# barlettacarmen/CrCNN

Hardware: NVIDIA B200
Metric: encrypted MNIST images/sec (higher is better)
Workload: dtype u64

## Files before the change

crcnn_b200/csrc/engine.cu:

```cuda
#include <cuda_runtime.h>
#include <dlfcn.h>
#include <algorithm>
#include <cstdlib>
#include <cstring>
#include <map>
#include <unordered_map>
#include <string>
#include <vector>

#include "../../include/crcnn_b200.h"
#include "kernels.cuh"
#include "params.h"
#include "tc_mac.cuh"
#include "tcn_mac.cuh"
#include "relin32.cuh"
#include "reenc.cuh"

using namespace crcnn;

namespace {

enum KernelClass {
    KC_NTT_FWD = 0, KC_NTT_INV, KC_MAC, KC_PLAIN_EXPAND, KC_POOL, KC_BN, KC_PLAIN_OP,
    KC_BEHZ_LIFT, KC_SQ_TENSOR, KC_BEHZ_FLOOR, KC_RELIN, KC_PROBE, KC_TC_SPLIT, KC_TC_MAC, KC_TCN_SPLIT, KC_TCN_MAC, KC_RELIN32, KC_REENC, KC_COUNT
// ... 1498 lines not shown
            e = launch_ntt_inv_tensor(ctx->dP, ctx->logn, ext, have_ntt ? src : nullptr, cur, KS, prod, fold, !lean, ctx->stream);
        }
        if (e == cudaSuccess) { ProfScope ps(ctx, KC_BEHZ_FLOOR, lp_bytes(ctx, (double)cur * 3 * (KS + ctx->K)),
                                                     (double)cur * 3 * n * (ctx->S * (ctx->K + 1) + ctx->S + ctx->K * ctx->S)); e = launch_behz_floor(ctx->hp.d, ctx->n, prod, cur, o->d + c0 * 3 * pw, ctx->stream, !lean); }
        if (e != cudaSuccess) rc = fail(ctx, CRCNN_ERR_CUDA, cudaGetErrorString(e));
    }
    dev_free(ctx, coef);
    dev_free(ctx, ext); dev_free(ctx, prod);
    if (rc) { crcnn_tensor_free(ctx, o); return rc; }
    *out3 = o;
    return CRCNN_OK;
}

int crcnn_relinearize(crcnn_ctx *ctx, crcnn_tensor *in3, crcnn_evk *evk, crcnn_tensor **out2) {
    if (!ctx) return CRCNN_ERR_INVALID_ARGUMENT;
    REQUIRE(in3 && evk && out2, "null argument");
    REQUIRE(in3->size == 3, "relinearize expects size-3 ciphertexts");
    int total_digits = 0;
    for (int i = 0; i < ctx->K; i++) {
        int bits = 0; for (uint64_t v = ctx->hp.d.tab[i].mod.q; v; v >>= 1) bits++;
        REQUIRE(evk->digits[i] * evk->dbc >= bits, "not enough evaluation keys");
        total_digits += evk->digits[i];
    }
    REQUIRE(total_digits <= 63, "too many key digits for 128-bit lazy accumulation");
    CU(cudaSetDevice(ctx->device));
    int rc = ensure_domain(ctx, in3, 0);
    if (rc) return rc;
    crcnn_tensor *o = nullptr;
    rc = new_tensor(ctx, in3->count, 2, 0, &o);
    if (rc) return rc;
    const size_t pw = poly_words(ctx);
    if (evk->has_r32 && ctx->relin_mode == 1) {
        const Relin32Consts &c = evk->r32.c;
        const size_t per_ct = relin32_scratch_bytes(ctx->n, ctx->K, c);
        const long step = std::max<long>(1, std::min<long>(std::min<long>(in3->count, 200000), (long)((2ull << 30) / per_ct)));
        void *scratch = nullptr;
        rc = dev_alloc(ctx, (size_t)step * per_ct, &scratch);
        if (rc) { crcnn_tensor_free(ctx, o); return rc; }
        for (long c0 = 0; c0 < in3->count && !rc; c0 += step) {
            const long cnt = std::min<long>(step, in3->count - c0);
            ProfScope ps(ctx, KC_RELIN32, lp_bytes(ctx, (double)cnt * 5 * ctx->K),
                         lp_bfly(ctx, (double)cnt * (c.D + 2 * ctx->K) * c.S3));
            cudaError_t e = relin32_run(ctx->dP, ctx->logn, ctx->K, evk->r32, in3->d + c0 * 3 * pw, o->d + c0 * 2 * pw, cnt, scratch, ctx->stream);
            if (e != cudaSuccess) rc = fail(ctx, CRCNN_ERR_CUDA, cudaGetErrorString(e));
        }
        dev_free(ctx, scratch);
        if (rc) { crcnn_tensor_free(ctx, o); return rc; }
        *out2 = o;
        return CRCNN_OK;
    }
    RelinArgs a{};
    a.evk = evk->d; a.dbc = evk->dbc;
    for (int i = 0; i < MAXK; i++) { a.key_off[i] = evk->key_off[i]; a.digits[i] = evk->digits[i]; }
    const size_t per_ct = (size_t)(1 + total_digits + 2) * pw * 8;
    const long step = std::max<long>(1, std::min<long>(in3->count, (long)((2ull << 30) / per_ct)));
    uint64_t *scratch = nullptr;
    rc = dev_alloc(ctx, (size_t)step * per_ct, (void **)&scratch);
    if (rc) { crcnn_tensor_free(ctx, o); return rc; }
    a.dsc = scratch;
    a.dig = scratch + (size_t)step * pw;
    a.acc = a.dig + (size_t)step * total_digits * pw;
    for (long c0 = 0; c0 < in3->count && !rc; c0 += step) {
        a.count = std::min<long>(step, in3->count - c0);
        a.in3 = in3->d + c0 * 3 * pw;
        a.out = o->d + c0 * 2 * pw;
        cudaError_t e;
        { ProfScope ps(ctx, KC_RELIN, lp_bytes(ctx, (double)a.count * 3 * ctx->K), lp_bfly(ctx, (double)a.count * total_digits * ctx->K)); e = launch_relin(ctx->dP, ctx->logn, ctx->K, a, ctx->stream); }
        if (e == cudaSuccess) {
            ProfScope ps(ctx, KC_NTT_INV, 2 * lp_bytes(ctx, (double)a.count * 2 * ctx->K) + lp_bytes(ctx, (double)a.count * 2 * ctx->K), lp_bfly(ctx, (double)a.count * 2 * ctx->K));
            e = launch_ntt_grouped(ctx->dP, ctx->logn, a.out, a.count * 2 * ctx->K, 0, ctx->K, true, ctx->K, 0, ctx->stream, a.acc, a.in3,
                                   2 * ctx->K, 3 * ctx->K);
        }
        if (e != cudaSuccess) rc = fail(ctx, CRCNN_ERR_CUDA, cudaGetErrorString(e));
    }
    dev_free(ctx, scratch);
    if (rc) { crcnn_tensor_free(ctx, o); return rc; }
// ... 476 lines not shown
```

crcnn_b200/csrc/relin32.cu:

```cuda
#include "relin32.cuh"
#include "kernels.cuh"
#include "devcfg.cuh"
#include "modarith.cuh"
#include <cmath>
#include <cstdlib>
#include <vector>

namespace crcnn {
namespace {

const uint32_t kAuxPrimes[R32_MAXP] = {1073643521u, 1073479681u, 1073184769u, 1073053697u};

uint32_t mulm(uint32_t a, uint32_t b, uint32_t p) { return (uint32_t)((uint64_t)a * b % p); }
uint32_t powm(uint32_t a, uint64_t e, uint32_t p) {
    uint32_t r = 1;
    for (; e; e >>= 1, a = mulm(a, a, p))
        if (e & 1) r = mulm(r, a, p);
    return r;
}
uint32_t invm(uint32_t a, uint32_t p) { return powm(a % p, p - 2, p); }
uint32_t shoup_companion(uint32_t w, uint32_t p) { return (uint32_t)(((uint64_t)w << 32) / p); }
uint32_t bitrev32(uint32_t v, int bits) {
    uint32_t r = 0;
    for (int i = 0; i < bits; i++) r |= ((v >> i) & 1u) << (bits - 1 - i);
// ... 108 lines not shown
    fwd_last_stage<NG, 3>(x, t4, p, twop, G);
    fwd_last_stage<NG, 4>(x, t4, p, twop, G);
}

template <int NG, int S>
__device__ __forceinline__ void inv_first_stage(uint32_t (&x)[32], const uint4 *__restrict__ t4, uint32_t p, uint32_t twop, int G) {
    constexpr int B = 5;
#pragma unroll
    for (int l2 = 0; l2 < (1 << (B - 2 - S)); l2++) {
        const uint4 W = __ldg(t4 + (16 - (16 >> S) + l2) * NG + G);
#pragma unroll
        for (int a = 0; a < (1 << S); a++) {
            const int i0 = ((2 * l2) << (S + 1)) + a, i1 = ((2 * l2 + 1) << (S + 1)) + a;
            gs32(x[i0], x[i0 + (1 << S)], W.x, W.y, p, twop);
            gs32(x[i1], x[i1 + (1 << S)], W.z, W.w, p, twop);
        }
    }
}

template <int NG>
__device__ __forceinline__ void inv_first32(uint32_t (&x)[32], const uint4 *__restrict__ t4, const uint2 *__restrict__ t1, uint32_t p,
                                            uint32_t twop, int G) {
    inv_first_stage<NG, 0>(x, t4, p, twop, G);
    inv_first_stage<NG, 1>(x, t4, p, twop, G);
    inv_first_stage<NG, 2>(x, t4, p, twop, G);
    inv_first_stage<NG, 3>(x, t4, p, twop, G);
    {
        const uint2 W = __ldg(t1 + G);
#pragma unroll
        for (int a = 0; a < 16; a++) gs32(x[a], x[a + 16], W.x, W.y, p, twop);
    }
}

template <int LOGN, int B, int GLOG, bool INV>
__device__ __forceinline__ void pass32(uint32_t *sm, const uint2 *__restrict__ tw, uint32_t p) {
    constexpr int N = 1 << LOGN, g = 1 << GLOG, TH = Plan32<LOGN>::THREADS;
    if constexpr (GLOG == 0) {
        static_assert(B == 5, "the contiguous pass takes 5 stages");
        constexpr int NG = N >> 5;
        const uint4 *t4 = reinterpret_cast<const uint4 *>(tw);
        const uint2 *t1 = tw + 30 * NG;
#pragma unroll 1
        for (int G = threadIdx.x; G < NG; G += TH) {
            uint4 *row = reinterpret_cast<uint4 *>(sm + G * 36);
            uint32_t x[32];
#pragma unroll
            for (int m = 0; m < 8; m++) {
                const uint4 v = row[m];
                x[4 * m] = v.x; x[4 * m + 1] = v.y; x[4 * m + 2] = v.z; x[4 * m + 3] = v.w;
            }
            if (INV) inv_first32<NG>(x, t4, t1, p, 2 * p, G);
            else fwd_last32<NG>(x, t4, t1, p, 2 * p, G);
#pragma unroll
            for (int m = 0; m < 8; m++) row[m] = make_uint4(x[4 * m], x[4 * m + 1], x[4 * m + 2], x[4 * m + 3]);
        }
    } else {
        static_assert(GLOG >= 5, "strided passes need gaps that are multiples of 32 words");
        constexpr int PSTR = g + (g >> 5) * 4;
#pragma unroll 1
        for (int G = threadIdx.x; G < (N >> B); G += TH) {
            const int blk = G >> GLOG, o = G & (g - 1);
            uint32_t *col = sm + pad32((blk << (GLOG + B)) + o);
            uint32_t x[1 << B];
#pragma unroll
            for (int k = 0; k < (1 << B); k++) x[k] = col[k * PSTR];
            if (INV) inv_group32<B>(x, tw, p, 2 * p, N >> (GLOG + 1), blk);
            else fwd_group32<B>(x, tw, p, 2 * p, (N >> (GLOG + B)) + blk);
#pragma unroll
            for (int k = 0; k < (1 << B); k++) col[k * PSTR] = x[k];
        }
    }
}

template <int LOGN>
__device__ __forceinline__ void ntt32_forward(uint32_t *sm, const uint2 *__restrict__ w, const uint2 *__restrict__ wl, uint32_t p) {
    using P = Plan32<LOGN>;
    constexpr int b0 = P::bits(0), b1 = P::NP > 1 ? P::bits(1) : 0;
    pass32<LOGN, b0, LOGN - b0, false>(sm, w, p);
    __syncthreads();
    if constexpr (P::NP > 1) {
        pass32<LOGN, b1, LOGN - b0 - b1, false>(sm, w, p);
        __syncthreads();
    }
    pass32<LOGN, 5, 0, false>(sm, wl, p);
    __syncthreads();
}

template <int LOGN>
__device__ __forceinline__ void ntt32_inverse(uint32_t *sm, const uint2 *__restrict__ iw, const uint2 *__restrict__ iwl, uint32_t p) {
    using P = Plan32<LOGN>;
    constexpr int b0 = P::bits(0), b1 = P::NP > 1 ? P::bits(1) : 0;
    pass32<LOGN, 5, 0, true>(sm, iwl, p);
    __syncthreads();
    if constexpr (P::NP > 1) {
        pass32<LOGN, b1, 5, true>(sm, iw, p);
        __syncthreads();
    }
    pass32<LOGN, b0, LOGN - b0, true>(sm, iw, p);
    __syncthreads();
}

template <int LOGN, int RANGE>
__device__ __forceinline__ void store32_canonical(const uint32_t *sm, uint32_t *__restrict__ dst, uint32_t p) {
    for (int i = threadIdx.x * 4; i < (1 << LOGN); i += Plan32<LOGN>::THREADS * 4) {
        uint4 v = *reinterpret_cast<const uint4 *>(sm + pad32(i));
        if (RANGE == 4) { v.x = csub(v.x, 2 * p); v.y = csub(v.y, 2 * p); v.z = csub(v.z, 2 * p); v.w = csub(v.w, 2 * p); }
        v.x = csub(v.x, p); v.y = csub(v.y, p); v.z = csub(v.z, p); v.w = csub(v.w, p);
        *reinterpret_cast<uint4 *>(dst + i) = v;
    }
}

__global__ void __launch_bounds__(256)
r32_scale_kernel(const DeviceParams *__restrict__ P, const Relin32Consts *__restrict__ cp, const uint64_t *__restrict__ in3,
                 uint16_t *__restrict__ planes) {
    const int n = P->n, K = P->K;
    const long pw = (long)K * n;
    const long ct = blockIdx.x;
    const long lw = ((long)blockIdx.y * 256 + threadIdx.x) * 2;
    const int i = (int)(lw / n), e = (int)(lw - (long)i * n);
    const ulonglong2 c2 = __ldg(reinterpret_cast<const ulonglong2 *>(in3 + (ct * 3 + 2) * pw + lw));
    const Mod mod = P->tab[i].mod;
    const uint64_t f = P->inv_qhat[i];
    const uint64_t v0 = mulmod(c2.x, f, mod), v1 = mulmod(c2.y, f, mod);
    const int dbc = cp->dbc, D = cp->D;
    const uint32_t mask = (1u << dbc) - 1;
    for (int d = cp->dfirst[i]; d < D && cp->dprime[d] == i; d++) {
        const int sh = cp->dshift[d];
        const uint32_t lo = (uint32_t)(v0 >> sh) & mask, hi = (uint32_t)(v1 >> sh) & mask;
        *reinterpret_cast<uint32_t *>(planes + (ct * D + d) * n + e) = lo | (hi << 16);
    }
}

template <int LOGN>
__global__ void __launch_bounds__(Plan32<LOGN>::THREADS, Plan32<LOGN>::MIN_CTAS)
r32_digits_kernel(const uint16_t *__restrict__ planes, const Relin32Consts *__restrict__ cp, uint32_t *__restrict__ dig) {
    extern __shared__ uint4 sm32v[];
    uint32_t *sm32 = reinterpret_cast<uint32_t *>(sm32v);
    constexpr int N = 1 << LOGN;
    const long b = blockIdx.x;
    const int S3 = cp->S3;
    const int s = (int)(b % S3);
    const long cd = b / S3;
    const uint32_t p = cp->p[s];
    const uint2 *w = cp->w[s];
    const uint16_t *src = planes + cd * N;
    for (int i = threadIdx.x * 8; i < N; i += Plan32<LOGN>::THREADS * 8) {
        const uint4 v = __ldg(reinterpret_cast<const uint4 *>(src + i));
        uint4 *dst = reinterpret_cast<uint4 *>(sm32 + pad32(i));
        dst[0] = make_uint4(v.x & 0xffffu, v.x >> 16, v.y & 0xffffu, v.y >> 16);
        dst[1] = make_uint4(v.z & 0xffffu, v.z >> 16, v.w & 0xffffu, v.w >> 16);
    }
    __syncthreads();
    ntt32_forward<LOGN>(sm32, w, cp->wl[s], p);
    store32_canonical<LOGN, 4>(sm32, dig + b * N, p);
}

struct KeyMap {
    long key_off[MAXK];
    uint32_t ninv[R32_MAXP];
};

template <int LOGN>
__global__ void __launch_bounds__(Plan32<LOGN>::THREADS, Plan32<LOGN>::MIN_CTAS)
r32_key_kernel(const uint64_t *__restrict__ coef, KeyMap km, const Relin32Consts *__restrict__ cp, int K, uint32_t *__restrict__ keys) {
    extern __shared__ uint4 sm32v[];
    uint32_t *sm32 = reinterpret_cast<uint32_t *>(sm32v);
    constexpr int N = 1 << LOGN;
    const long b = blockIdx.x;
    const int S3 = cp->S3, D = cp->D;
    const int s = (int)(b % S3);
    const int o = (int)((b / S3) % (2 * K));
    const int d = (int)(b / ((long)S3 * 2 * K));
    const int pi = o / K, j = o % K;
    const uint32_t p = cp->p[s];
    const uint64_t *src = coef + km.key_off[cp->dprime[d]] + ((long)(2 * (cp->dshift[d] / cp->dbc) + pi) * K + j) * N;
    for (int e = threadIdx.x; e < N; e += blockDim.x) sm32[pad32(e)] = (uint32_t)(__ldg(src + e) % p);
    __syncthreads();
    ntt32_forward<LOGN>(sm32, cp->w[s], cp->wl[s], p);
    uint32_t *dst = keys + (((long)s * D + d) * 2 * K + o) * N;
    const uint32_t ninv = km.ninv[s];
    for (int e = threadIdx.x; e < N; e += blockDim.x) {
        const uint32_t v = csub(csub(sm32[pad32(e)], 2 * p), p);
        dst[e] = (uint32_t)((uint64_t)v * ninv % p);
    }
}

__device__ __forceinline__ uint32_t red64_32(uint64_t x, uint64_t mu, uint32_t p) {
    const uint32_t r = (uint32_t)x - (uint32_t)__umul64hi(x, mu) * p;
    return csub(csub(r, 2 * p), p);
}
__device__ __forceinline__ void madwide(uint64_t &acc, uint32_t a, uint32_t b) {
    asm("mad.wide.u32 %0, %1, %2, %0;" : "+l"(acc) : "r"(a), "r"(b));
}

template <int T, int OC, int EW>
__global__ void __launch_bounds__(256)
r32_mac_kernel(const uint32_t *__restrict__ dig, const uint32_t *__restrict__ keys, const Relin32Consts *__restrict__ cp, int n,
               long count, int cpb, uint32_t *__restrict__ acc) {
    extern __shared__ uint4 sm32v[];
    uint32_t *ksm = reinterpret_cast<uint32_t *>(sm32v);
    constexpr int LANES = 256 / EW;
    const int el = threadIdx.x % EW, lane = threadIdx.x / EW;
    const int e = blockIdx.x * EW + el;
    const int s = blockIdx.y;
    const long ctb = (long)blockIdx.z * cpb;
    const long cte = min(ctb + cpb, count);
    const uint32_t p = cp->p[s];
    const uint64_t mu = cp->mu[s];
    const int D = cp->D, S3 = cp->S3;
    {
        const uint32_t *kg = keys + (long)s * D * OC * n + blockIdx.x * EW;
// ... 114 lines not shown
#pragma unroll
                for (int u = 0; u < CPS; u++) {
                    a[u][0] = red64_32(a[u][0], mu, p);
                    a[u][1] = red64_32(a[u][1], mu, p);
                }
            }
        }
#pragma unroll
        for (int u = 0; u < CPS; u++) {
            const long ct = ctb + (long)st * CPS + u;
            if (ct < cte) {
                uint32_t *ap = acc + ((ct * OC + og * 2) * S3 + s) * n + e0 + el;
                ap[0] = red64_32(a[u][0], mu, p);
                ap[(long)S3 * n] = red64_32(a[u][1], mu, p);
            }
        }
    }
}

template <int LOGN>
__global__ void __launch_bounds__(Plan32<LOGN>::THREADS, Plan32<LOGN>::MIN_CTAS)
r32_intt_kernel(const Relin32Consts *__restrict__ cp, uint32_t *__restrict__ acc) {
    extern __shared__ uint4 sm32v[];
    uint32_t *sm32 = reinterpret_cast<uint32_t *>(sm32v);
    constexpr int N = 1 << LOGN;
    const long b = blockIdx.x;
    const int s = (int)(b % cp->S3);
    const uint32_t p = cp->p[s];
    const uint2 *iw = cp->iw[s];
    uint32_t *poly = acc + b * N;
    for (int i = threadIdx.x * 4; i < N; i += Plan32<LOGN>::THREADS * 4)
        *reinterpret_cast<uint4 *>(sm32 + pad32(i)) = *reinterpret_cast<const uint4 *>(poly + i);
    __syncthreads();
    ntt32_inverse<LOGN>(sm32, iw, cp->iwl[s], p);
    store32_canonical<LOGN, 2>(sm32, poly, p);
}

struct CrtConsts {
    uint32_t p[R32_MAXP], half[R32_MAXP], ginv[R32_MAXP][R32_MAXP], ginvp[R32_MAXP][R32_MAXP];
    uint64_t c[R32_MAXP], csh[R32_MAXP], Pmodq, q;
};
template <int S3>
__device__ __forceinline__ uint64_t crt_one(const uint32_t (&r)[R32_MAXP], const CrtConsts &k) {
    uint32_t a[S3];
#pragma unroll
    for (int s = 0; s < S3; s++) {
        uint32_t t = r[s];
#pragma unroll
        for (int i = 0; i < s; i++) {
            const uint32_t ai = csub(a[i], k.p[s]);
            t = csub(shoup32(t + k.p[s] - ai, k.ginv[s][i], k.ginvp[s][i], k.p[s]), k.p[s]);
        }
        a[s] = t;
    }
    uint64_t v = a[0];
    bool neg = false, decided = false;
#pragma unroll
    for (int s = S3 - 1; s >= 0; s--) {
        if (s > 0) v += mulshoup_lazy((uint64_t)a[s], k.c[s], k.csh[s], k.q);
        if (!decided && a[s] != k.half[s]) { neg = a[s] > k.half[s]; decided = true; }
    }
    v = v >= 4 * k.q ? v - 4 * k.q : v;
    v = v >= 2 * k.q ? v - 2 * k.q : v;
    v = v >= k.q ? v - k.q : v;
    if (neg) v = submod(v, k.Pmodq, k.q);
    return v;
}

template <int S3>
__global__ void __launch_bounds__(256)
r32_crt_kernel(const DeviceParams *__restrict__ P, const Relin32Consts *__restrict__ cp, const uint32_t *__restrict__ acc,
               const uint64_t *__restrict__ in3, uint64_t *__restrict__ out) {
    const int n = P->n, K = P->K;
    const int e = (blockIdx.y * 256 + threadIdx.x) * 2;
    const int o = (int)(blockIdx.x % (unsigned)(2 * K));
    const long ct = blockIdx.x / (unsigned)(2 * K);
    const int pi = o / K, j = o % K;
    CrtConsts k;
#pragma unroll
    for (int s = 0; s < S3; s++) {
        k.p[s] = cp->p[s];
        k.half[s] = cp->half[s];
        k.c[s] = cp->cmodq[j][s];
        k.csh[s] = cp->cmodq_sh[j][s];
#pragma unroll
        for (int i = 0; i < s; i++) {
            k.ginv[s][i] = cp->ginv[s][i];
            k.ginvp[s][i] = cp->ginvp[s][i];
        }
    }
    k.Pmodq = cp->Pmodq[j];
    k.q = P->tab[j].mod.q;
    const uint32_t *r = acc + ((ct * 2 * K + o) * S3) * n + e;
    uint32_t r0[R32_MAXP], r1[R32_MAXP];
#pragma unroll
    for (int s = 0; s < S3; s++) {
        const uint2 v = __ldg(reinterpret_cast<const uint2 *>(r + (long)s * n));
        r0[s] = v.x;
        r1[s] = v.y;
    }
    const long w = (long)j * n + e;
    const ulonglong2 c = __ldg(reinterpret_cast<const ulonglong2 *>(in3 + (ct * 3 + pi) * (long)K * n + w));
    ulonglong2 res;
    res.x = addmod(c.x, crt_one<S3>(r0, k), k.q);
    res.y = addmod(c.y, crt_one<S3>(r1, k), k.q);
    *reinterpret_cast<ulonglong2 *>(out + (ct * 2 + pi) * (long)K * n + w) = res;
}

template <int LOGN, int S3>
__global__ void __launch_bounds__(Plan32<LOGN>::THREADS, 2)
r32_intt_crt_kernel(const DeviceParams *__restrict__ P, const Relin32Consts *__restrict__ cp, const uint32_t *__restrict__ acc,
                    const uint64_t *__restrict__ in3, uint64_t *__restrict__ out) {
    extern __shared__ uint4 sm32v[];
    uint32_t *sm32 = reinterpret_cast<uint32_t *>(sm32v);
    constexpr int N = 1 << LOGN, SW = Plan32<LOGN>::SMEM_WORDS;
    const int K = P->K;
    const long b = blockIdx.x;
    const int o = (int)(b % (2 * K));
    const long ct = b / (2 * K);
    const int pi = o / K, j = o % K;
#pragma unroll
    for (int s = 0; s < S3; s++) {
        const uint32_t *poly = acc + (b * S3 + s) * N;
        for (int i = threadIdx.x * 4; i < N; i += Plan32<LOGN>::THREADS * 4)
            *reinterpret_cast<uint4 *>(sm32 + s * SW + pad32(i)) = __ldg(reinterpret_cast<const uint4 *>(poly + i));
    }
    __syncthreads();
#pragma unroll
    for (int s = 0; s < S3; s++) ntt32_inverse<LOGN>(sm32 + s * SW, cp->iw[s], cp->iwl[s], cp->p[s]);
    CrtConsts k;
#pragma unroll
    for (int s = 0; s < S3; s++) {
        k.p[s] = cp->p[s];
        k.half[s] = cp->half[s];
        k.c[s] = cp->cmodq[j][s];
        k.csh[s] = cp->cmodq_sh[j][s];
#pragma unroll
        for (int i = 0; i < s; i++) {
            k.ginv[s][i] = cp->ginv[s][i];
            k.ginvp[s][i] = cp->ginvp[s][i];
        }
    }
    k.Pmodq = cp->Pmodq[j];
    k.q = P->tab[j].mod.q;
    const uint64_t *cin = in3 + (ct * 3 + pi) * (long)K * N + (long)j * N;
    uint64_t *dst = out + (ct * 2 + pi) * (long)K * N + (long)j * N;
    for (int e = threadIdx.x * 2; e < N; e += Plan32<LOGN>::THREADS * 2) {
        uint32_t r0[R32_MAXP], r1[R32_MAXP];
#pragma unroll
        for (int s = 0; s < S3; s++) {
            const uint2 v = *reinterpret_cast<const uint2 *>(sm32 + s * SW + pad32(e));
            r0[s] = csub(v.x, k.p[s]);
            r1[s] = csub(v.y, k.p[s]);
        }
        const ulonglong2 c = __ldg(reinterpret_cast<const ulonglong2 *>(cin + e));
        ulonglong2 res;
        res.x = addmod(c.x, crt_one<S3>(r0, k), k.q);
        res.y = addmod(c.y, crt_one<S3>(r1, k), k.q);
        *reinterpret_cast<ulonglong2 *>(dst + e) = res;
    }
}

template <int LOGN>
void configure32() {
    static DeviceOnce once;
    if (!once.first()) return;
    const int smem = Plan32<LOGN>::SMEM_WORDS * 4;
    cudaFuncSetAttribute(r32_digits_kernel<LOGN>, cudaFuncAttributeMaxDynamicSharedMemorySize, smem);
    cudaFuncSetAttribute(r32_key_kernel<LOGN>, cudaFuncAttributeMaxDynamicSharedMemorySize, smem);
    cudaFuncSetAttribute(r32_intt_kernel<LOGN>, cudaFuncAttributeMaxDynamicSharedMemorySize, smem);
    cudaFuncSetAttribute(r32_digits_kernel<LOGN>, cudaFuncAttributePreferredSharedMemoryCarveout, cudaSharedmemCarveoutMaxShared);
    cudaFuncSetAttribute(r32_intt_kernel<LOGN>, cudaFuncAttributePreferredSharedMemoryCarveout, cudaSharedmemCarveoutMaxShared);
}

template <int T, int OC, int EW>
cudaError_t launch_mac(const uint32_t *dig, const Relin32 &r, int n, long count, int cpb, unsigned gz, size_t bytes_per_coeff, uint32_t *acc,
                       cudaStream_t stream) {
    const size_t smem = bytes_per_coeff * EW;
    cudaError_t e = cudaFuncSetAttribute(r32_mac_kernel<T, OC, EW>, cudaFuncAttributeMaxDynamicSharedMemorySize, (int)smem);
    if (e != cudaSuccess) return e;
    r32_mac_kernel<T, OC, EW><<<dim3((unsigned)(n / EW), (unsigned)r.c.S3, gz), 256, smem, stream>>>(dig, r.keys, r.dc, n, count, cpb, acc);
    return cudaGetLastError();
}

template <int D, int OC>
cudaError_t launch_mac_reg(const uint32_t *dig, const Relin32 &r, int n, long count, int cpb, unsigned gz, uint32_t *acc, cudaStream_t stream) {
    constexpr size_t smem = (size_t)6 * 2 * D * 64 * 4;
    static DeviceOnce once;
    if (once.first()) {
        cudaError_t e = cudaFuncSetAttribute(r32_mac_reg_kernel<D, OC>, cudaFuncAttributeMaxDynamicSharedMemorySize, (int)smem);
        if (e != cudaSuccess) return e;
        cudaFuncSetAttribute(r32_mac_reg_kernel<D, OC>, cudaFuncAttributePreferredSharedMemoryCarveout, cudaSharedmemCarveoutMaxShared);
    }
    r32_mac_reg_kernel<D, OC><<<dim3((unsigned)(n / 64), (unsigned)r.c.S3, gz), 32 * OC, smem, stream>>>(dig, r.keys, r.dc, n, count, cpb, acc);
    return cudaGetLastError();
}

template <int LOGN>
cudaError_t run_t(const DeviceParams *dP, int K, const Relin32 &r, const uint64_t *in3, uint64_t *out, long count, void *scratch,
                  cudaStream_t stream) {
    using Pl = Plan32<LOGN>;
    constexpr int N = 1 << LOGN;
    configure32<LOGN>();
    const Relin32Consts &c = r.c;
    const size_t smem = Pl::SMEM_WORDS * 4;
    uint32_t *dig = (uint32_t *)scratch;
    uint32_t *acc = dig + (size_t)count * c.D * c.S3 * N;
    uint16_t *planes = (uint16_t *)(acc + (size_t)count * 2 * K * c.S3 * N);
    r32_scale_kernel<<<dim3((unsigned)count, (unsigned)((long)K * N / 512)), 256, 0, stream>>>(dP, r.dc, in3, planes);
    r32_digits_kernel<LOGN><<<(unsigned)(count * c.D * c.S3), Pl::THREADS, smem, stream>>>(planes, r.dc, dig);
    {
        const int cpb = 128;
        const unsigned gz = (unsigned)((count + cpb - 1) / cpb);
        const size_t ksmem = (size_t)c.D * 2 * K * 4;
        cudaError_t e = cudaSuccess;
        const bool generic = std::getenv("CRCNN_R32_GENERIC_MAC") != nullptr;
        if (!generic && c.D == 4 * K && K == 1) e = launch_mac_reg<4, 2>(dig, r, N, count, cpb, gz, acc, stream);
        else if (!generic && c.D == 4 * K && K == 2) e = launch_mac_reg<8, 4>(dig, r, N, count, cpb, gz, acc, stream);
        else if (!generic && c.D == 4 * K && K == 4) e = launch_mac_reg<16, 8>(dig, r, N, count, cpb, gz, acc, stream);
        else if (!generic && c.D == 4 * K && K == 8) e = launch_mac_reg<32, 16>(dig, r, N, count, cpb, gz, acc, stream);
        else
        switch (2 * K) {
            case 2: e = launch_mac<4, 2, 64>(dig, r, N, count, cpb, gz, ksmem, acc, stream); break;
            case 4: e = launch_mac<4, 4, 64>(dig, r, N, count, cpb, gz, ksmem, acc, stream); break;
            case 8: e = launch_mac<4, 8, 64>(dig, r, N, count, cpb, gz, ksmem, acc, stream); break;
            case 16: e = launch_mac<2, 16, 32>(dig, r, N, count, cpb, gz, ksmem, acc, stream); break;
            default: e = cudaErrorInvalidValue;
        }
        if (e != cudaSuccess) return e;
    }
    if constexpr (LOGN <= 13) {
        static const bool fused = !(std::getenv("CRCNN_R32_FUSED") && std::atoi(std::getenv("CRCNN_R32_FUSED")) == 0);
        if (fused && c.S3 == 3) {
            static DeviceOnce once3;
            const int smem3 = 3 * Pl::SMEM_WORDS * 4;
            if (once3.first()) {
                cudaFuncSetAttribute(r32_intt_crt_kernel<LOGN, 3>, cudaFuncAttributeMaxDynamicSharedMemorySize, smem3);
                cudaFuncSetAttribute(r32_intt_crt_kernel<LOGN, 3>, cudaFuncAttributePreferredSharedMemoryCarveout, cudaSharedmemCarveoutMaxShared);
            }
            r32_intt_crt_kernel<LOGN, 3><<<(unsigned)(count * 2 * K), Pl::THREADS, smem3, stream>>>(dP, r.dc, acc, in3, out);
            return cudaGetLastError();
        }
    }
    r32_intt_kernel<LOGN><<<(unsigned)(count * 2 * K * c.S3), Pl::THREADS, smem, stream>>>(r.dc, acc);
    const dim3 gc((unsigned)(count * 2 * K), (unsigned)(N / 512));
    if (c.S3 == 2) r32_crt_kernel<2><<<gc, 256, 0, stream>>>(dP, r.dc, acc, in3, out);
    else if (c.S3 == 3) r32_crt_kernel<3><<<gc, 256, 0, stream>>>(dP, r.dc, acc, in3, out);
    else r32_crt_kernel<4><<<gc, 256, 0, stream>>>(dP, r.dc, acc, in3, out);
    return cudaGetLastError();
}

template <int LOGN>
cudaError_t build_keys_t(const uint64_t *coef, const KeyMap &km, const Relin32 &r, int K, cudaStream_t stream) {
    configure32<LOGN>();
    r32_key_kernel<LOGN><<<(unsigned)((long)r.c.D * 2 * K * r.c.S3), Plan32<LOGN>::THREADS, Plan32<LOGN>::SMEM_WORDS * 4, stream>>>(
        coef, km, r.dc, K, r.keys);
    return cudaGetLastError();
}

}

bool relin32_applicable(int n, int K, const uint64_t *q, const int *digits, int dbc, Relin32Consts &c) {
    if (n < 1024 || n > 16384 || (n & (n - 1))) return false;
    if (dbc < 1 || dbc > 16) return false;
    if (K != 1 && K != 2 && K != 4 && K != 8) return false;
    c = Relin32Consts{};
    c.dbc = dbc;
    uint64_t qmax = 0;
    for (int i = 0; i < K; i++) {
        if (q[i] > qmax) qmax = q[i];
        c.dfirst[i] = c.D;
        for (int k = 0; k < digits[i]; k++) {
            if (c.D >= 32) return false;
            c.dprime[c.D] = (unsigned char)i;
            c.dshift[c.D] = (unsigned char)(k * dbc);
            c.D++;
        }
    }
    if (c.D == 0) return false;
    const double need = 1.0 + std::log2((double)c.D) + std::log2((double)n) + (double)dbc + std::log2((double)qmax);
    double have = 0;
    for (int s = 0; s < R32_MAXP; s++) {
        have += std::log2((double)kAuxPrimes[s]);
        if (have > need + 1e-3 && s + 1 >= 2) { c.S3 = s + 1; break; }
    }
    if (c.S3 == 0) return false;
    for (int s = 0; s < c.S3; s++) {
        c.p[s] = kAuxPrimes[s];
        c.mu[s] = (uint64_t)((((unsigned __int128)1) << 64) / kAuxPrimes[s]);
        c.half[s] = (kAuxPrimes[s] - 1) / 2;
        for (int k = 0; k < s; k++) {
            c.ginv[s][k] = invm(kAuxPrimes[k] % kAuxPrimes[s], kAuxPrimes[s]);
            c.ginvp[s][k] = shoup_companion(c.ginv[s][k], kAuxPrimes[s]);
        }
    }
    for (int j = 0; j < K; j++) {
        unsigned __int128 prod = 1;
        for (int s = 0; s < c.S3; s++) {
            c.cmodq[j][s] = (uint64_t)prod;
            c.cmodq_sh[j][s] = (uint64_t)((prod << 64) / q[j]);
            prod = prod * kAuxPrimes[s] % q[j];
        }
        c.Pmodq[j] = (uint64_t)prod;
    }
    return true;
}

cudaError_t relin32_build(const DeviceParams *dP, int logn, int K, const uint64_t *q, const uint64_t *evk_dev, const long *key_off,
                          long total_polys, Relin32 &r, cudaStream_t stream) {
    (void)q;
    const int n = 1 << logn;
    Relin32Consts &c = r.c;
    std::vector<uint2> host((size_t)4 * c.S3 * n);
    const int NG = n >> 5;
    KeyMap km{};
    for (int s = 0; s < c.S3; s++) {
        const uint32_t p = c.p[s];
        uint32_t psi = 0;
        for (uint32_t z = 2; z < 1000 && !psi; z++) {
            const uint32_t cand = powm(z, (p - 1) / (2u * n), p);
            if (powm(cand, n, p) == p - 1) psi = cand;
        }
        if (!psi) return cudaErrorInvalidValue;
        const uint32_t psi_inv = invm(psi, p);
        uint32_t pw = 1, ipw = 1;
        uint2 *w = host.data() + (size_t)(4 * s) * n, *iw = w + n, *wl = iw + n, *iwl = wl + n;
        for (int i = 0; i < n; i++) {
// ... 41 lines not shown
    if (e != cudaSuccess) return e;
    const size_t words = (size_t)total_polys * K * n;
    uint64_t *coef = nullptr;
    e = cudaMalloc((void **)&coef, words * 8);
    if (e != cudaSuccess) return e;
    e = cudaMalloc((void **)&r.keys, (size_t)c.S3 * c.D * 2 * K * n * 4);
    if (e != cudaSuccess) { cudaFree(coef); return e; }
    e = cudaMemcpyAsync(coef, evk_dev, words * 8, cudaMemcpyDeviceToDevice, stream);
    if (e == cudaSuccess) e = launch_ntt(dP, logn, coef, total_polys * K, 0, K, true, stream);
    if (e == cudaSuccess) {
        switch (logn) {
            case 10: e = build_keys_t<10>(coef, km, r, K, stream); break;
            case 11: e = build_keys_t<11>(coef, km, r, K, stream); break;
            case 12: e = build_keys_t<12>(coef, km, r, K, stream); break;
            case 13: e = build_keys_t<13>(coef, km, r, K, stream); break;
            case 14: e = build_keys_t<14>(coef, km, r, K, stream); break;
            default: e = cudaErrorInvalidValue;
        }
    }
    if (e == cudaSuccess) e = cudaStreamSynchronize(stream);
    cudaFree(coef);
    return e;
}

void relin32_free(Relin32 &r) {
    if (r.keys) cudaFree(r.keys);
    if (r.tables) cudaFree(r.tables);
    if (r.dc) cudaFree(r.dc);
    r.dc = nullptr;
    r.keys = nullptr;
    r.tables = nullptr;
}

size_t relin32_scratch_bytes(int n, int K, const Relin32Consts &c) {
    return (size_t)c.D * c.S3 * n * 4 + (size_t)2 * K * c.S3 * n * 4 + (size_t)c.D * n * 2;
}

cudaError_t relin32_run(const DeviceParams *dP, int logn, int K, const Relin32 &r, const uint64_t *in3, uint64_t *out, long count,
                        void *scratch, cudaStream_t stream) {
    if (count <= 0) return cudaSuccess;
    switch (logn) {
        case 10: return run_t<10>(dP, K, r, in3, out, count, scratch, stream);
        case 11: return run_t<11>(dP, K, r, in3, out, count, scratch, stream);
        case 12: return run_t<12>(dP, K, r, in3, out, count, scratch, stream);
        case 13: return run_t<13>(dP, K, r, in3, out, count, scratch, stream);
        case 14: return run_t<14>(dP, K, r, in3, out, count, scratch, stream);
        default: return cudaErrorInvalidValue;
    }
}

}
```

crcnn_b200/csrc/relin32.cuh:

```cuda
#pragma once
#include <cuda_runtime.h>
#include <cstdint>
#include "params.h"

namespace crcnn {

constexpr int R32_MAXP = 4;

struct Relin32Consts {
    int S3;
    int D;
    int dbc;
    uint32_t p[R32_MAXP];
    uint64_t mu[R32_MAXP];
    const uint2 *w[R32_MAXP];
    const uint2 *iw[R32_MAXP];
    const uint2 *wl[R32_MAXP], *iwl[R32_MAXP];
    uint32_t ginv[R32_MAXP][R32_MAXP];
    uint32_t ginvp[R32_MAXP][R32_MAXP];
    uint32_t half[R32_MAXP];
    uint64_t cmodq[MAXK][R32_MAXP];
    uint64_t cmodq_sh[MAXK][R32_MAXP];
    uint64_t Pmodq[MAXK];
    unsigned char dprime[32], dshift[32];
    int dfirst[MAXK];
};

struct Relin32 {
    Relin32Consts c;
    uint32_t *keys = nullptr;
    uint2 *tables = nullptr;
    Relin32Consts *dc = nullptr;
};

bool relin32_applicable(int n, int K, const uint64_t *q, const int *digits, int dbc, Relin32Consts &c);

cudaError_t relin32_build(const DeviceParams *dP, int logn, int K, const uint64_t *q, const uint64_t *evk_dev, const long *key_off,
                          long total_polys, Relin32 &r, cudaStream_t stream);
void relin32_free(Relin32 &r);

size_t relin32_scratch_bytes(int n, int K, const Relin32Consts &c);

cudaError_t relin32_run(const DeviceParams *dP, int logn, int K, const Relin32 &r, const uint64_t *in3, uint64_t *out, long count,
                        void *scratch, cudaStream_t stream);

}
```

Measured before the change: 39.54.

## Fuse digit scaling into per-digit NTT kernel and split 3-prime iNTT across warp groups

Adds a v2 relinearization path, enabled by default and switchable with an environment variable. The scale kernel is fused into a new digits kernel that extracts one digit plane into shared memory and reuses it for the forward NTT under every auxiliary prime, which removes the 16-bit planes round trip through global memory and the extra launch. The 3-prime inverse NTT plus CRT kernel now runs the three prime NTTs concurrently in separate thread groups synchronized by named barriers, instead of running them one after another with the whole block. The cost is fewer CTAs in the digits grid with more work each, plus extra shared memory per block.

```diff
diff --git a/crcnn_b200/csrc/engine.cu b/crcnn_b200/csrc/engine.cu
--- a/crcnn_b200/csrc/engine.cu
+++ b/crcnn_b200/csrc/engine.cu
@@ -1554,7 +1554,8 @@
     const size_t pw = poly_words(ctx);
     if (evk->has_r32 && ctx->relin_mode == 1) {
         const Relin32Consts &c = evk->r32.c;
-        const size_t per_ct = relin32_scratch_bytes(ctx->n, ctx->K, c);
+        const bool v2 = relin32_v2();
+        const size_t per_ct = relin32_scratch_bytes(ctx->n, ctx->K, c, v2);
         const long step = std::max<long>(1, std::min<long>(std::min<long>(in3->count, 200000), (long)((2ull << 30) / per_ct)));
         void *scratch = nullptr;
         rc = dev_alloc(ctx, (size_t)step * per_ct, &scratch);
@@ -1563,7 +1564,8 @@
             const long cnt = std::min<long>(step, in3->count - c0);
             ProfScope ps(ctx, KC_RELIN32, lp_bytes(ctx, (double)cnt * 5 * ctx->K),
                          lp_bfly(ctx, (double)cnt * (c.D + 2 * ctx->K) * c.S3));
-            cudaError_t e = relin32_run(ctx->dP, ctx->logn, ctx->K, evk->r32, in3->d + c0 * 3 * pw, o->d + c0 * 2 * pw, cnt, scratch, ctx->stream);
+            cudaError_t e = relin32_run(ctx->dP, ctx->logn, ctx->K, evk->r32, in3->d + c0 * 3 * pw, o->d + c0 * 2 * pw, cnt, v2, scratch,
+                                         ctx->stream);
             if (e != cudaSuccess) rc = fail(ctx, CRCNN_ERR_CUDA, cudaGetErrorString(e));
         }
         dev_free(ctx, scratch);
diff --git a/crcnn_b200/csrc/relin32.cu b/crcnn_b200/csrc/relin32.cu
--- a/crcnn_b200/csrc/relin32.cu
+++ b/crcnn_b200/csrc/relin32.cu
@@ -164,16 +164,25 @@
     }
 }
 
-template <int LOGN, int B, int GLOG, bool INV>
-__device__ __forceinline__ void pass32(uint32_t *sm, const uint2 *__restrict__ tw, uint32_t p) {
-    constexpr int N = 1 << LOGN, g = 1 << GLOG, TH = Plan32<LOGN>::THREADS;
+struct CtaBar {
+    __device__ __forceinline__ void sync() const { __syncthreads(); }
+};
+template <int TH>
+struct GroupBar {
+    int id;
+    __device__ __forceinline__ void sync() const { asm volatile("bar.sync %0, %1;" ::"r"(id), "n"(TH) : "memory"); }
+};
+
+template <int LOGN, int B, int GLOG, bool INV, int TH>
+__device__ __forceinline__ void pass32(uint32_t *sm, const uint2 *__restrict__ tw, uint32_t p, int tid, const uint16_t *in16 = nullptr) {
+    constexpr int N = 1 << LOGN, g = 1 << GLOG;
     if constexpr (GLOG == 0) {
         static_assert(B == 5, "the contiguous pass takes 5 stages");
         constexpr int NG = N >> 5;
         const uint4 *t4 = reinterpret_cast<const uint4 *>(tw);
         const uint2 *t1 = tw + 30 * NG;
 #pragma unroll 1
-        for (int G = threadIdx.x; G < NG; G += TH) {
+        for (int G = tid; G < NG; G += TH) {
             uint4 *row = reinterpret_cast<uint4 *>(sm + G * 36);
             uint32_t x[32];
 #pragma unroll
@@ -190,12 +199,18 @@
         static_assert(GLOG >= 5, "strided passes need gaps that are multiples of 32 words");
         constexpr int PSTR = g + (g >> 5) * 4;
 #pragma unroll 1
-        for (int G = threadIdx.x; G < (N >> B); G += TH) {
+        for (int G = tid; G < (N >> B); G += TH) {
             const int blk = G >> GLOG, o = G & (g - 1);
             uint32_t *col = sm + pad32((blk << (GLOG + B)) + o);
             uint32_t x[1 << B];
-#pragma unroll
-            for (int k = 0; k < (1 << B); k++) x[k] = col[k * PSTR];
+            if (!INV && in16) {
+                const uint16_t *c16 = in16 + (blk << (GLOG + B)) + o;
+#pragma unroll
+                for (int k = 0; k < (1 << B); k++) x[k] = c16[k * g];
+            } else {
+#pragma unroll
+                for (int k = 0; k < (1 << B); k++) x[k] = col[k * PSTR];
+            }
             if (INV) inv_group32<B>(x, tw, p, 2 * p, N >> (GLOG + 1), blk);
             else fwd_group32<B>(x, tw, p, 2 * p, (N >> (GLOG + B)) + blk);
 #pragma unroll
@@ -204,32 +219,34 @@
     }
 }
 
-template <int LOGN>
-__device__ __forceinline__ void ntt32_forward(uint32_t *sm, const uint2 *__restrict__ w, const uint2 *__restrict__ wl, uint32_t p) {
+template <int LOGN, int TH = Plan32<LOGN>::THREADS, class Bar = CtaBar>
+__device__ __forceinline__ void ntt32_forward(uint32_t *sm, const uint2 *__restrict__ w, const uint2 *__restrict__ wl, uint32_t p, int tid,
+                                              Bar bar = {}, const uint16_t *in16 = nullptr) {
     using P = Plan32<LOGN>;
     constexpr int b0 = P::bits(0), b1 = P::NP > 1 ? P::bits(1) : 0;
-    pass32<LOGN, b0, LOGN - b0, false>(sm, w, p);
-    __syncthreads();
+    pass32<LOGN, b0, LOGN - b0, false, TH>(sm, w, p, tid, in16);
+    bar.sync();
     if constexpr (P::NP > 1) {
-        pass32<LOGN, b1, LOGN - b0 - b1, false>(sm, w, p);
-        __syncthreads();
-    }
-    pass32<LOGN, 5, 0, false>(sm, wl, p);
-    __syncthreads();
-}
-
-template <int LOGN>
-__device__ __forceinline__ void ntt32_inverse(uint32_t *sm, const uint2 *__restrict__ iw, const uint2 *__restrict__ iwl, uint32_t p) {
+        pass32<LOGN, b1, LOGN - b0 - b1, false, TH>(sm, w, p, tid);
+        bar.sync();
+    }
+    pass32<LOGN, 5, 0, false, TH>(sm, wl, p, tid);
+    bar.sync();
+}
+
+template <int LOGN, int TH = Plan32<LOGN>::THREADS, class Bar = CtaBar>
+__device__ __forceinline__ void ntt32_inverse(uint32_t *sm, const uint2 *__restrict__ iw, const uint2 *__restrict__ iwl, uint32_t p, int tid,
+                                              Bar bar = {}) {
     using P = Plan32<LOGN>;
     constexpr int b0 = P::bits(0), b1 = P::NP > 1 ? P::bits(1) : 0;
-    pass32<LOGN, 5, 0, true>(sm, iwl, p);
-    __syncthreads();
+    pass32<LOGN, 5, 0, true, TH>(sm, iwl, p, tid);
+    bar.sync();
     if constexpr (P::NP > 1) {
-        pass32<LOGN, b1, 5, true>(sm, iw, p);
-        __syncthreads();
-    }
-    pass32<LOGN, b0, LOGN - b0, true>(sm, iw, p);
-    __syncthreads();
+        pass32<LOGN, b1, 5, true, TH>(sm, iw, p, tid);
+        bar.sync();
+    }
+    pass32<LOGN, b0, LOGN - b0, true, TH>(sm, iw, p, tid);
+    bar.sync();
 }
 
 template <int LOGN, int RANGE>
@@ -283,8 +300,46 @@
         dst[1] = make_uint4(v.z & 0xffffu, v.z >> 16, v.w & 0xffffu, v.w >> 16);
     }
     __syncthreads();
-    ntt32_forward<LOGN>(sm32, w, cp->wl[s], p);
+    ntt32_forward<LOGN>(sm32, w, cp->wl[s], p, threadIdx.x);
     store32_canonical<LOGN, 4>(sm32, dig + b * N, p);
+}
+
+template <int LOGN>
+__global__ void __launch_bounds__(Plan32<LOGN>::THREADS, Plan32<LOGN>::MIN_CTAS)
+r32_digits_c2_kernel(const DeviceParams *__restrict__ P, const Relin32Consts *__restrict__ cp, const uint64_t *__restrict__ in3,
+                     uint32_t *__restrict__ dig) {
+    extern __shared__ uint4 sm32v[];
+    uint32_t *sm32 = reinterpret_cast<uint32_t *>(sm32v);
+    constexpr int N = 1 << LOGN, TH = Plan32<LOGN>::THREADS;
+    uint16_t *plane = reinterpret_cast<uint16_t *>(sm32 + Plan32<LOGN>::SMEM_WORDS);
+    const long b = blockIdx.x;
+    const int D = cp->D, S3 = cp->S3;
+    const long ct = b / D;
+    const int d = (int)(b - ct * D);
+    const int i = cp->dprime[d], sh = cp->dshift[d];
+    const uint32_t mask = (1u << cp->dbc) - 1;
+    const uint64_t q = P->tab[i].mod.q, f = P->inv_qhat[i], fsh = cp->inv_qhat_sh[i];
+    auto digit = [&](uint64_t x) {
+        uint64_t v = mulshoup_lazy(x, f, fsh, q);
+        v = v >= q ? v - q : v;
+        return (uint32_t)(v >> sh) & mask;
+    };
+    const uint64_t *src = in3 + (ct * 3 + 2) * (long)P->K * N + (long)i * N;
+    for (int e = threadIdx.x * 8; e < N; e += TH * 8) {
+        uint32_t w[4];
+#pragma unroll
+        for (int k = 0; k < 4; k++) {
+            const ulonglong2 c = __ldg(reinterpret_cast<const ulonglong2 *>(src + e + 2 * k));
+            w[k] = digit(c.x) | (digit(c.y) << 16);
+        }
+        *reinterpret_cast<uint4 *>(plane + e) = make_uint4(w[0], w[1], w[2], w[3]);
+    }
+    for (int s = 0; s < S3; s++) {
+        __syncthreads();
+        const uint32_t p = cp->p[s];
+        ntt32_forward<LOGN>(sm32, cp->w[s], cp->wl[s], p, threadIdx.x, CtaBar{}, plane);
+        store32_canonical<LOGN, 4>(sm32, dig + (b * S3 + s) * N, p);
+    }
 }
 
 struct KeyMap {
@@ -308,7 +363,7 @@
     const uint64_t *src = coef + km.key_off[cp->dprime[d]] + ((long)(2 * (cp->dshift[d] / cp->dbc) + pi) * K + j) * N;
     for (int e = threadIdx.x; e < N; e += blockDim.x) sm32[pad32(e)] = (uint32_t)(__ldg(src + e) % p);
     __syncthreads();
-    ntt32_forward<LOGN>(sm32, cp->w[s], cp->wl[s], p);
+    ntt32_forward<LOGN>(sm32, cp->w[s], cp->wl[s], p, threadIdx.x);
     uint32_t *dst = keys + (((long)s * D + d) * 2 * K + o) * N;
     const uint32_t ninv = km.ninv[s];
     for (int e = threadIdx.x; e < N; e += blockDim.x) {
@@ -489,7 +544,7 @@
     for (int i = threadIdx.x * 4; i < N; i += Plan32<LOGN>::THREADS * 4)
         *reinterpret_cast<uint4 *>(sm32 + pad32(i)) = *reinterpret_cast<const uint4 *>(poly + i);
     __syncthreads();
-    ntt32_inverse<LOGN>(sm32, iw, cp->iwl[s], p);
+    ntt32_inverse<LOGN>(sm32, iw, cp->iwl[s], p, threadIdx.x);
     store32_canonical<LOGN, 2>(sm32, poly, p);
 }
 
@@ -497,6 +552,26 @@
     uint32_t p[R32_MAXP], half[R32_MAXP], ginv[R32_MAXP][R32_MAXP], ginvp[R32_MAXP][R32_MAXP];
     uint64_t c[R32_MAXP], csh[R32_MAXP], Pmodq, q;
 };
+template <int S3>
+__device__ __forceinline__ CrtConsts crt_consts(const DeviceParams *__restrict__ P, const Relin32Consts *__restrict__ cp, int j) {
+    CrtConsts k;
+#pragma unroll
+    for (int s = 0; s < S3; s++) {
+        k.p[s] = cp->p[s];
+        k.half[s] = cp->half[s];
+        k.c[s] = cp->cmodq[j][s];
+        k.csh[s] = cp->cmodq_sh[j][s];
+#pragma unroll
+        for (int i = 0; i < s; i++) {
+            k.ginv[s][i] = cp->ginv[s][i];
+            k.ginvp[s][i] = cp->ginvp[s][i];
+        }
+    }
+    k.Pmodq = cp->Pmodq[j];
+    k.q = P->tab[j].mod.q;
+    return k;
+}
+
 template <int S3>
 __device__ __forceinline__ uint64_t crt_one(const uint32_t (&r)[R32_MAXP], const CrtConsts &k) {
     uint32_t a[S3];
@@ -533,21 +608,7 @@
     const int o = (int)(blockIdx.x % (unsigned)(2 * K));
     const long ct = blockIdx.x / (unsigned)(2 * K);
     const int pi = o / K, j = o % K;
-    CrtConsts k;
-#pragma unroll
-    for (int s = 0; s < S3; s++) {
-        k.p[s] = cp->p[s];
-        k.half[s] = cp->half[s];
-        k.c[s] = cp->cmodq[j][s];
-        k.csh[s] = cp->cmodq_sh[j][s];
-#pragma unroll
-        for (int i = 0; i < s; i++) {
-            k.ginv[s][i] = cp->ginv[s][i];
-            k.ginvp[s][i] = cp->ginvp[s][i];
-        }
-    }
-    k.Pmodq = cp->Pmodq[j];
-    k.q = P->tab[j].mod.q;
+    const CrtConsts k = crt_consts<S3>(P, cp, j);
     const uint32_t *r = acc + ((ct * 2 * K + o) * S3) * n + e;
     uint32_t r0[R32_MAXP], r1[R32_MAXP];
 #pragma unroll
@@ -584,22 +645,8 @@
     }
     __syncthreads();
 #pragma unroll
-    for (int s = 0; s < S3; s++) ntt32_inverse<LOGN>(sm32 + s * SW, cp->iw[s], cp->iwl[s], cp->p[s]);
-    CrtConsts k;
-#pragma unroll
-    for (int s = 0; s < S3; s++) {
-        k.p[s] = cp->p[s];
-        k.half[s] = cp->half[s];
-        k.c[s] = cp->cmodq[j][s];
-        k.csh[s] = cp->cmodq_sh[j][s];
-#pragma unroll
-        for (int i = 0; i < s; i++) {
-            k.ginv[s][i] = cp->ginv[s][i];
-            k.ginvp[s][i] = cp->ginvp[s][i];
-        }
-    }
-    k.Pmodq = cp->Pmodq[j];
-    k.q = P->tab[j].mod.q;
+    for (int s = 0; s < S3; s++) ntt32_inverse<LOGN>(sm32 + s * SW, cp->iw[s], cp->iwl[s], cp->p[s], threadIdx.x);
+    const CrtConsts k = crt_consts<S3>(P, cp, j);
     const uint64_t *cin = in3 + (ct * 3 + pi) * (long)K * N + (long)j * N;
     uint64_t *dst = out + (ct * 2 + pi) * (long)K * N + (long)j * N;
     for (int e = threadIdx.x * 2; e < N; e += Plan32<LOGN>::THREADS * 2) {
@@ -614,6 +661,50 @@
         ulonglong2 res;
         res.x = addmod(c.x, crt_one<S3>(r0, k), k.q);
         res.y = addmod(c.y, crt_one<S3>(r1, k), k.q);
+        *reinterpret_cast<ulonglong2 *>(dst + e) = res;
+    }
+}
+
+template <int LOGN>
+constexpr int R32_GT3 = Plan32<LOGN>::THREADS / 2 < 32 ? 32 : Plan32<LOGN>::THREADS / 2;
+template <int LOGN, int GT = R32_GT3<LOGN>>
+__global__ void __launch_bounds__(3 * GT, 768 / (3 * GT))
+r32_intt_crt3_kernel(const DeviceParams *__restrict__ P, const Relin32Consts *__restrict__ cp, const uint32_t *__restrict__ acc,
+                     const uint64_t *__restrict__ in3, uint64_t *__restrict__ out) {
+    extern __shared__ uint4 sm32v[];
+    uint32_t *sm32 = reinterpret_cast<uint32_t *>(sm32v);
+    constexpr int N = 1 << LOGN, SW = Plan32<LOGN>::SMEM_WORDS;
+    const int K = P->K;
+    const long b = blockIdx.x;
+    const int o = (int)(b % (2 * K));
+    const long ct = b / (2 * K);
+    const int pi = o / K, j = o % K;
+    const int g = threadIdx.x / GT, tid = threadIdx.x % GT;
+    {
+        uint32_t *sg = sm32 + g * SW;
+        const uint32_t *poly = acc + (b * 3 + g) * N;
+        for (int i = tid * 4; i < N; i += GT * 4)
+            *reinterpret_cast<uint4 *>(sg + pad32(i)) = __ldg(reinterpret_cast<const uint4 *>(poly + i));
+        const GroupBar<GT> bar{1 + g};
+        bar.sync();
+        ntt32_inverse<LOGN, GT>(sg, cp->iw[g], cp->iwl[g], cp->p[g], tid, bar);
+    }
+    __syncthreads();
+    const CrtConsts k = crt_consts<3>(P, cp, j);
+    const uint64_t *cin = in3 + (ct * 3 + pi) * (long)K * N + (long)j * N;
+    uint64_t *dst = out + (ct * 2 + pi) * (long)K * N + (long)j * N;
+    for (int e = threadIdx.x * 2; e < N; e += 3 * GT * 2) {
+        uint32_t r0[R32_MAXP], r1[R32_MAXP];
+#pragma unroll
+        for (int s = 0; s < 3; s++) {
+            const uint2 v = *reinterpret_cast<const uint2 *>(sm32 + s * SW + pad32(e));
+            r0[s] = csub(v.x, k.p[s]);
+            r1[s] = csub(v.y, k.p[s]);
+        }
+        const ulonglong2 c = __ldg(reinterpret_cast<const ulonglong2 *>(cin + e));
+        ulonglong2 res;
+        res.x = addmod(c.x, crt_one<3>(r0, k), k.q);
+        res.y = addmod(c.y, crt_one<3>(r1, k), k.q);
         *reinterpret_cast<ulonglong2 *>(dst + e) = res;
     }
 }
@@ -628,6 +719,8 @@
     cudaFuncSetAttribute(r32_intt_kernel<LOGN>, cudaFuncAttributeMaxDynamicSharedMemorySize, smem);
     cudaFuncSetAttribute(r32_digits_kernel<LOGN>, cudaFuncAttributePreferredSharedMemoryCarveout, cudaSharedmemCarveoutMaxShared);
     cudaFuncSetAttribute(r32_intt_kernel<LOGN>, cudaFuncAttributePreferredSharedMemoryCarveout, cudaSharedmemCarveoutMaxShared);
+    cudaFuncSetAttribute(r32_digits_c2_kernel<LOGN>, cudaFuncAttributeMaxDynamicSharedMemorySize, smem + (1 << LOGN) * 2);
+    cudaFuncSetAttribute(r32_digits_c2_kernel<LOGN>, cudaFuncAttributePreferredSharedMemoryCarveout, cudaSharedmemCarveoutMaxShared);
 }
 
 template <int T, int OC, int EW>
@@ -654,7 +747,7 @@
 }
 
 template <int LOGN>
-cudaError_t run_t(const DeviceParams *dP, int K, const Relin32 &r, const uint64_t *in3, uint64_t *out, long count, void *scratch,
+cudaError_t run_t(const DeviceParams *dP, int K, const Relin32 &r, const uint64_t *in3, uint64_t *out, long count, bool v2, void *scratch,
                   cudaStream_t stream) {
     using Pl = Plan32<LOGN>;
     constexpr int N = 1 << LOGN;
@@ -663,9 +756,13 @@
     const size_t smem = Pl::SMEM_WORDS * 4;
     uint32_t *dig = (uint32_t *)scratch;
     uint32_t *acc = dig + (size_t)count * c.D * c.S3 * N;
-    uint16_t *planes = (uint16_t *)(acc + (size_t)count * 2 * K * c.S3 * N);
-    r32_scale_kernel<<<dim3((unsigned)count, (unsigned)((long)K * N / 512)), 256, 0, stream>>>(dP, r.dc, in3, planes);
-    r32_digits_kernel<LOGN><<<(unsigned)(count * c.D * c.S3), Pl::THREADS, smem, stream>>>(planes, r.dc, dig);
+    if (v2) {
+        r32_digits_c2_kernel<LOGN><<<(unsigned)(count * c.D), Pl::THREADS, smem + N * 2, stream>>>(dP, r.dc, in3, dig);
+    } else {
+        uint16_t *planes = (uint16_t *)(acc + (size_t)count * 2 * K * c.S3 * N);
+        r32_scale_kernel<<<dim3((unsigned)count, (unsigned)((long)K * N / 512)), 256, 0, stream>>>(dP, r.dc, in3, planes);
+        r32_digits_kernel<LOGN><<<(unsigned)(count * c.D * c.S3), Pl::THREADS, smem, stream>>>(planes, r.dc, dig);
+    }
     {
         const int cpb = 128;
         const unsigned gz = (unsigned)((count + cpb - 1) / cpb);
@@ -694,8 +791,11 @@
             if (once3.first()) {
                 cudaFuncSetAttribute(r32_intt_crt_kernel<LOGN, 3>, cudaFuncAttributeMaxDynamicSharedMemorySize, smem3);
                 cudaFuncSetAttribute(r32_intt_crt_kernel<LOGN, 3>, cudaFuncAttributePreferredSharedMemoryCarveout, cudaSharedmemCarveoutMaxShared);
-            }
-            r32_intt_crt_kernel<LOGN, 3><<<(unsigned)(count * 2 * K), Pl::THREADS, smem3, stream>>>(dP, r.dc, acc, in3, out);
+                cudaFuncSetAttribute(r32_intt_crt3_kernel<LOGN>, cudaFuncAttributeMaxDynamicSharedMemorySize, smem3);
+                cudaFuncSetAttribute(r32_intt_crt3_kernel<LOGN>, cudaFuncAttributePreferredSharedMemoryCarveout, cudaSharedmemCarveoutMaxShared);
+            }
+            if (v2) r32_intt_crt3_kernel<LOGN><<<(unsigned)(count * 2 * K), 3 * R32_GT3<LOGN>, smem3, stream>>>(dP, r.dc, acc, in3, out);
+            else r32_intt_crt_kernel<LOGN, 3><<<(unsigned)(count * 2 * K), Pl::THREADS, smem3, stream>>>(dP, r.dc, acc, in3, out);
             return cudaGetLastError();
         }
     }
@@ -750,6 +850,15 @@
             c.ginv[s][k] = invm(kAuxPrimes[k] % kAuxPrimes[s], kAuxPrimes[s]);
             c.ginvp[s][k] = shoup_companion(c.ginv[s][k], kAuxPrimes[s]);
         }
+    }
+    for (int i = 0; i < K; i++) {
+        unsigned __int128 qh = 1;
+        for (int j = 0; j < K; j++)
+            if (j != i) qh = qh * (q[j] % q[i]) % q[i];
+        unsigned __int128 inv = 1, b = qh;
+        for (uint64_t e = q[i] - 2; e; e >>= 1, b = b * b % q[i])
+            if (e & 1) inv = inv * b % q[i];
+        c.inv_qhat_sh[i] = (uint64_t)((inv << 64) / q[i]);
     }
     for (int j = 0; j < K; j++) {
         unsigned __int128 prod = 1;
@@ -857,19 +966,24 @@
     r.tables = nullptr;
 }
 
-size_t relin32_scratch_bytes(int n, int K, const Relin32Consts &c) {
-    return (size_t)c.D * c.S3 * n * 4 + (size_t)2 * K * c.S3 * n * 4 + (size_t)c.D * n * 2;
-}
-
-cudaError_t relin32_run(const DeviceParams *dP, int logn, int K, const Relin32 &r, const uint64_t *in3, uint64_t *out, long count,
+bool relin32_v2() {
+    const char *v = std::getenv("CRCNN_R32_V2");
+    return !(v && std::atoi(v) == 0);
+}
+
+size_t relin32_scratch_bytes(int n, int K, const Relin32Consts &c, bool v2) {
+    return (size_t)c.D * c.S3 * n * 4 + (size_t)2 * K * c.S3 * n * 4 + (v2 ? 0 : (size_t)c.D * n * 2);
+}
+
+cudaError_t relin32_run(const DeviceParams *dP, int logn, int K, const Relin32 &r, const uint64_t *in3, uint64_t *out, long count, bool v2,
                         void *scratch, cudaStream_t stream) {
     if (count <= 0) return cudaSuccess;
     switch (logn) {
-        case 10: return run_t<10>(dP, K, r, in3, out, count, scratch, stream);
-        case 11: return run_t<11>(dP, K, r, in3, out, count, scratch, stream);
-        case 12: return run_t<12>(dP, K, r, in3, out, count, scratch, stream);
-        case 13: return run_t<13>(dP, K, r, in3, out, count, scratch, stream);
-        case 14: return run_t<14>(dP, K, r, in3, out, count, scratch, stream);
+        case 10: return run_t<10>(dP, K, r, in3, out, count, v2, scratch, stream);
+        case 11: return run_t<11>(dP, K, r, in3, out, count, v2, scratch, stream);
+        case 12: return run_t<12>(dP, K, r, in3, out, count, v2, scratch, stream);
+        case 13: return run_t<13>(dP, K, r, in3, out, count, v2, scratch, stream);
+        case 14: return run_t<14>(dP, K, r, in3, out, count, v2, scratch, stream);
         default: return cudaErrorInvalidValue;
     }
 }
diff --git a/crcnn_b200/csrc/relin32.cuh b/crcnn_b200/csrc/relin32.cuh
--- a/crcnn_b200/csrc/relin32.cuh
+++ b/crcnn_b200/csrc/relin32.cuh
@@ -22,6 +22,7 @@
     uint64_t cmodq[MAXK][R32_MAXP];
     uint64_t cmodq_sh[MAXK][R32_MAXP];
     uint64_t Pmodq[MAXK];
+    uint64_t inv_qhat_sh[MAXK];
     unsigned char dprime[32], dshift[32];
     int dfirst[MAXK];
 };
@@ -39,9 +40,11 @@
                           long total_polys, Relin32 &r, cudaStream_t stream);
 void relin32_free(Relin32 &r);
 
-size_t relin32_scratch_bytes(int n, int K, const Relin32Consts &c);
+bool relin32_v2();
 
-cudaError_t relin32_run(const DeviceParams *dP, int logn, int K, const Relin32 &r, const uint64_t *in3, uint64_t *out, long count,
+size_t relin32_scratch_bytes(int n, int K, const Relin32Consts &c, bool v2);
+
+cudaError_t relin32_run(const DeviceParams *dP, int logn, int K, const Relin32 &r, const uint64_t *in3, uint64_t *out, long count, bool v2,
                         void *scratch, cudaStream_t stream);
 
 }
```

After: 40.07, median of 6. 1.3% higher.
